# Peterande/SAST

Measured on AMD Instinct MI355X. Metric: frames/sec (B=4) SAST backbone fwd+bwd, 1Mpx 640x360, higher is better.
Workload: dtype f32; 1 GPU; 1Mpx 640x360 (padded 384x640) full SAST backbone + PAFPN, fwd+bwd + AdamW, B=4/GPU, binary events (rand>0.5), random-init, AMP=0.0002; global_batch=4, seq_len=1, parallelism=dp1, hipgraph=True, library=sast_amd/libsast_hip.so, product_library=True, segmented_backward_overlap=False, deferred_weight_gradients=False, backward_cuts=3, dw_discard_TIMING_PROBE_gradients_invalid=False, collective_ranks=1, collective_ranks_verified=1, gradient_bytes_per_rank=67663616, sync_batchnorm=False, event_dtype=int32, grads_finite=True

## Files before the change

### include/sast_hip.h

```cpp
#ifndef SAST_HIP_H
#define SAST_HIP_H
#include <stddef.h>
#include <stdint.h>

#ifdef __cplusplus
extern "C" {
#endif

typedef void* sast_stream_t;

enum { SAST_DT_F32 = 0, SAST_DT_I32 = 1, SAST_DT_U8 = 2, SAST_DT_I64 = 3, SAST_DT_I16 = 4, SAST_DT_I8 = 5 };

int sast_version(void);
int sast_mfma_split3(void);

int sast_nzratio(const void* x, int dtype, int B, int Cin, int H, int W, int32_t* cnt_ws, float* r, sast_stream_t stream);
int sast_nzratio_padded(const void* x, int dtype, int B, int Cin, int H, int W, int Hp, int Wp, int32_t* cnt_ws, float* r,
                        sast_stream_t stream);

int sast_input_prep(const void* x, int dtype, int B, int C, int H, int W, int Hp, int Wp, int32_t* ws, float* r, float* y,
                    sast_stream_t stream);
int sast_input_prep_flag(const void* x, int dtype, int B, int C, int H, int W, int Hp, int Wp, int32_t* ws, float* r, float* y,
                         uint32_t* nonexact, sast_stream_t stream);
int sast_input_prep_u8(const uint8_t* x, int B, int C, int H, int W, int Hp, int Wp, int32_t* ws, float* r, uint8_t* y, sast_stream_t stream);
// ... 33 lines not shown
typedef struct SastScoreArgs {
  int32_t B, L, C, r_stride;
  float amp;
  const float* xp;
  const float* r;
  const float* ws_w; const float* ws_b;
  const float* wc;
  float* scale;
  float* s;
  float* xw;
  float* tok;
  const float* dxw; float* dxp;
  float* d_ws_w; float* d_ws_b; float* d_wc;
  float* ws;
  float* dscale_ws;
} SastScoreArgs;
int sast_score_stp_fwd(const SastScoreArgs* a, sast_stream_t stream);
int sast_score_stp_bwd(const SastScoreArgs* a, sast_stream_t stream);

typedef struct SastSel {
  int32_t* win_keep;
  uint64_t* mask;
  int32_t* K;
  int32_t* row_off;
  int32_t* win_rank;
  int32_t* counts;
  int32_t* tok_slot;
  int32_t* row_tok;
  int32_t* pack_rows;
  int32_t* row_seg;
// ... 18 lines not shown
  float *mean1, *rstd1;
  float *mean2, *rstd2;
  float *S, *QKV, *O, *lse, *Y, *UG, *Hh;
  const float* dout; float* dxin;
  float *d_ln1_w, *d_ln1_b, *d_ln2_w, *d_ln2_b, *d_qkv_w, *d_qkv_b, *d_proj_w, *d_proj_b, *d_ls1;
  float *d_fc1_w, *d_fc1_b, *d_fc2_w, *d_fc2_b, *d_ls2;
  float* ws;
  float *cb_m, *cb_sum;
  float* raw_ws;
  const float *drop1, *drop2;
  float* drop_ws;
  const float* drop_mlp;
  float* fused_ws;
  const float* act_w;
  float* d_act_w;
} SastMswsaArgs;
size_t sast_mswsa_fused_ws_floats(int C, int inner, int T, int dim_head, int cb_tps);
size_t sast_mswsa_raw_ws_floats(int C, int inner);
size_t sast_mswsa_bwd_ws_floats(int rows, int C, int inner);
int sast_mswsa_fwd(const SastMswsaArgs* a, sast_stream_t stream);
int sast_mswsa_bwd(const SastMswsaArgs* a, sast_stream_t stream);

typedef struct SastLstmArgs {
  int32_t B, L, C;
  const float* x; const float* h0; const float* c0;
  const float* w; const float* b;
  float* h1; float* c1;
  float* gates;
  const float* dh1; const float* dc1;
  float* dx; float* dh0; float* dc0;
// ... 399 lines not shown
```

### sast_amd/csrc/k_block.hip

```cpp
#include <cstdlib>
#include "gemm_dispatch.cuh"
#include "kernels.h"

using namespace sast;

namespace {

constexpr int ATTN_MAX_T = 256;

struct EpBiasRelu {
  float* c; int ldc; const float* bias;
  struct Col { float b; };
  using Aux = EpNone;
  __device__ __forceinline__ Col col(int j) const { return Col{bias[j]}; }
  __device__ __forceinline__ Aux pre(int, int) const { return Aux{}; }
  __device__ __forceinline__ void post(int m, int j, const float (&v)[1], const Col& k, const Aux&) const {
    c[(size_t)m * ldc + j] = fmaxf(v[0] + k.b, 0.f);
  }
};
struct EpBiasReluCtl : EpBiasRelu {
  static constexpr bool SIDE = true;
  ControlsJob k; int side_blocks;
  __device__ __forceinline__ void side(int sb) const { if (threadIdx.x < 256) controls_fwd_elem(k, sb * 256 + threadIdx.x); }
};
// ... 297 lines not shown
  EpBiasReluCtl ep{};
  ep.c = a->s; ep.ldc = C; ep.bias = a->ws_b;
  ep.k = ControlsJob{a->wc, a->r, a->r_stride, a->scale, a->dscale_ws, nullptr, nullptr, a->B, C, 20};
  ep.side_blocks = (a->B * C + 255) / 256;
  int rc = gemm_auto(LdRows{a->xp, C, nullptr}, LdWeightNT{a->ws_w, C, 0}, ep, M, C, C, nullptr, st);
  if (rc) return rc;
  return stp_fwd_launch(a->xp, a->s, a->scale, a->amp, a->xw, a->tok, a->B, a->L, C, st);
}

int sast_score_stp_bwd(const SastScoreArgs* a, sast_stream_t stream) { SAST_ENTRY();
  hipStream_t st = (hipStream_t)stream;
  ProfScope ps_("score_bwd", a->C, a->B * a->L, st);
  const int M = a->B * a->L, C = a->C;
  float* dz = a->ws;
  float* dscale = a->dscale_ws ? a->dscale_ws : a->ws + (size_t)M * C;
  if (!a->dscale_ws) zero_fill(dscale, sizeof(float) * a->B * C, st);
  int rc = stp_bwd_launch(a->xp, a->s, a->scale, a->dxw, a->dxp, dz, dscale, a->B, a->L, C, st);
  if (rc) return rc;
  EpStoreAddCtl ep{};
  ep.c = a->dxp; ep.ldc = C; ep.add = a->dxp; ep.ldadd = C;
  ep.k = ControlsJob{a->wc, a->r, a->r_stride, nullptr, nullptr, dscale, a->d_wc, a->B, C, 20};
  ep.side_blocks = (C * 20 + 255) / 256;
  return gemm_pair(LdRowsT{dz, C}, LdRowsT{a->xp, C}, a->d_ws_w, C, C, C, M, nullptr, a->d_ws_b,
                   LdRows{dz, C, nullptr}, LdWeightNN{a->ws_w, C}, ep, M, C, C, nullptr, st);
}

size_t sast_mswsa_fused_ws_floats(int C, int inner, int T, int dim_head, int cb_tps) {
  const int on = SAST_KNOB("SAST_MSWSA_FUSED", 1);
  if (!on || !mswsa_fused_supported(C, inner, T, dim_head > 0 ? dim_head : 32, cb_tps)) return 0;
  return mswsa_fused_plane_floats(C, inner);
}
size_t sast_mswsa_raw_ws_floats(int C, int inner) { return (size_t)C * inner + (size_t)C * C + 2 * C; }

// ... 52 lines not shown
  if (!a->cb_m || !a->cb_sum || R % a->cb_tps) return SAST_EINVAL;
  rc = gemm_auto(LdRows{a->Hh, inner, nullptr}, LdWeightNT{a->fc2_w, inner, 0}, EpStore{a->cb_m, C, a->fc2_b}, R, C, inner, dR, st);
  if (rc) return rc;
  rc = cb_sample_sum_launch(a->cb_m, C, false, a->sel.row_tok, dR, R, a->cb_tps, R / a->cb_tps, C, a->cb_sum, st);
  if (rc) return rc;
  return cb_apply_fwd_launch(a->cb_m, a->Y, a->ls2, a->cb_sum, a->sel.row_tok, dR, R, a->cb_tps, C, a->out, st, a->drop2);
}

int sast_mswsa_bwd(const SastMswsaArgs* a, sast_stream_t stream) { SAST_ENTRY();
  hipStream_t st = (hipStream_t)stream;
  ProfScope ps_("mswsa_bwd", a->C, (a->mode ? -1 : 1) * a->B * a->H * a->W, st);
  const int C = a->C, L = a->H * a->W, R = a->B * L, inner = a->inner;
  const int T = a->ph * a->pw, NW = a->B * (L / T);
  const int dh = a->dim_head > 0 ? a->dim_head : 32;
  if (T > ATTN_MAX_T || a->mlp_act < 0 || a->mlp_act >= GLU_ACT_COUNT) return SAST_EINVAL;
  const int* dR = a->sel.counts;
  const int* row_tok = a->sel.row_tok;
  float* dUG = a->ws;
  float* dY = dUG + (size_t)R * 2 * inner;
  float* dO = dY + (size_t)R * C;
  float* dQKV = dO + (size_t)R * C;
  float* dS = dQKV + (size_t)R * 3 * C;
  float* raw2 = a->raw_ws ? a->raw_ws : dS + (size_t)R * C;
  float* raw1 = raw2 + (size_t)C * inner;
  float* s2 = raw1 + (size_t)C * C;
  float* s1 = s2 + C;
  if (!a->raw_ws) zero_fill(raw2, sizeof(float) * sast_mswsa_raw_ws_floats(C, inner), st);
  int rc;
  const float* dz = a->dout;
  const int* dz_tok = row_tok;
// ... 54 lines not shown
    rc = gemm_tn(LdRowsT{dYb, C}, LdRowsT{a->O, C}, raw1, C, C, C, R, dR, s1, st);
    if (rc) return rc;
    rc = gemm_auto(LdRows{dYb, C, nullptr}, LdWeightNN{a->proj_w, C}, EpStore{dO, C, nullptr}, R, C, C, dR, st);
  }
  if (rc) return rc;
  {
    const LsFinish f2{a->fc2_w, a->fc2_b, a->ls2, raw2, s2, a->d_fc2_w, a->d_fc2_b, a->d_ls2, inner};
    const LsFinish f1{a->proj_w, a->proj_b, a->ls1, raw1, s1, a->d_proj_w, a->d_proj_b, a->d_ls1, C};
    rc = attn_bwd_mfma_launch(a->QKV, dO, a->lse, dQKV, a->sel.row_off, a->sel.K, NW, T, C, dh, st, &f2, &f1, C,
                              a->ws + mswsa_bwd_ws_base(R, C, inner));
  }
  if (rc) return rc;
  rc = gemm_pair(LdRowsT{dQKV, 3 * C}, LdRowsT{a->S, C}, a->d_qkv_w, C, 3 * C, C, R, dR, a->d_qkv_b,
                 LdRows{dQKV, 3 * C, nullptr}, LdWeightNN{a->qkv_w, C}, EpStoreAdd{dS, C, dY, C}, R, C, 3 * C, dR, st);
  if (rc) return rc;
  return ln1_gather_bwd_launch(a->xin, a->dout, dS, a->sel.tok_slot, a->ln1_w, a->ln1_b, a->ln2_w, a->mean1, a->rstd1, a->mean2,
                               a->rstd2, a->dxin, a->d_ln1_w, a->d_ln1_b, a->d_ln2_w, a->d_ln2_b, R, C, st);
}

int sast_lstm_fwd(const SastLstmArgs* a, sast_stream_t stream) { SAST_ENTRY();
  hipStream_t st = (hipStream_t)stream;
  ProfScope ps_("lstm_fwd", a ? a->C : 0, a ? a->B * a->L : 0, st);
  if (!a || a->C % 4) return SAST_EINVAL;
  const int M = a->B * a->L, C = a->C;
  const int Kred = a->h0 ? 2 * C : C;
  const LdRows2 la{a->x, C, C, a->h0, C};
  const LdWeightNT lb{a->w, 2 * C, C};
  const EpLstm ep{a->b, a->c0, a->h1, a->c1, a->gates, C, a->drop};
  const int mode = SAST_KNOB("SAST_LSTM_TILE", 0);
  const bool k4 = mode && Kred >= 256 && (long)((M + 63) / 64) * ((C + 31) / 32) <= 2 * pair_thin_nb();
// ... 37 lines not shown
```

### sast_amd/csrc/k_rows.hip

```cpp
#include <cstdlib>
#include "common.cuh"
#include "kernels.h"

namespace sast {

__global__ __launch_bounds__(256) void zero_fill_kernel(float* __restrict__ p, size_t n) {
  const size_t i = (size_t)blockIdx.x * 256 + threadIdx.x;
  if (i < n) p[i] = 0.f;
}
int zero_fill(void* p, size_t bytes, hipStream_t st) {
  const size_t n = (bytes + 3) / 4;
  if (!n) return SAST_OK;
  SAST_LAUNCH(zero_fill_kernel, dim3((unsigned)((n + 255) / 256)), dim3(256), 0, st, (float*)p, n);
  SAST_CHECK_LAUNCH();
  return SAST_OK;
}

template <typename T>
__global__ __launch_bounds__(256) void nzr_count_kernel(const T* __restrict__ x, int* __restrict__ cnt, int C, int H, int W) {
  __shared__ float cell[8][33];
  const int plane = blockIdx.z;
  const int cy = threadIdx.x >> 5, cx = threadIdx.x & 31;
  const int y0 = blockIdx.y * 32 + cy * 4;
  int n1 = 0, n2 = 0, n3 = 0, n4 = 0;
// ... 450 lines not shown
    case 512: { constexpr int GL = 64, VPL = 2; CALL; } break;  \
    case 1024:{ constexpr int GL = 64, VPL = 4; CALL; } break;  \
    default: return SAST_EINVAL;                      \
  }

static int row_width_rc(int C) {
  SAST_DISPATCH_C(C, (void)(GL + VPL));
  return SAST_OK;
}
bool row_width_supported(int C) { return row_width_rc(C) == SAST_OK; }

static inline int bwd_grid(int rows, int rpb) {
  const int cap = SAST_KNOB("SAST_LN_BLOCKS", 256);
  int g = (rows + rpb - 1) / rpb;
  return g < 1 ? 1 : (g > cap ? cap : g);
}

int ln_fwd_launch(const float* x, float* y, const float* gamma, const float* beta, const float* add, int add_rows,
                  float* mean, float* rstd, int rows, int C, float eps, hipStream_t st) {
  if (rows <= 0) return SAST_OK;
  SAST_DISPATCH_C(C, SAST_LAUNCH((ln_fwd_kernel<GL, VPL>), dim3((rows + 256 / GL - 1) / (256 / GL)), dim3(256), 0, st,
                                        x, y, gamma, beta, add, add_rows, mean, rstd, rows, eps));
  SAST_CHECK_LAUNCH();
  return SAST_OK;
}

int ln_bwd_launch(const float* x, const float* dy, const float* gamma, const float* mean, const float* rstd, float* dx,
                  float* dgamma, float* dbeta, int rows, int C, hipStream_t st) {
  if (rows <= 0) return SAST_OK;
  SAST_DISPATCH_C(C, SAST_LAUNCH((ln_bwd_kernel<GL, VPL>), dim3(bwd_grid(rows, ROWB / GL)), dim3(ROWB),
// ... 20 lines not shown
  IO::load(xin + (size_t)row * IO::C, v, gl);
  IO::load(g1, gm, gl);
  IO::load(b1, bt, gl);
  float mean, rstd;
  ln_row<GL, VPL>(v, gm, bt, eps, mean, rstd);
  if (gl == 0) { mean1[row] = mean; rstd1[row] = rstd; }
  const int slot = tok_slot[row];
  if (slot < 0) { IO::store(out + (size_t)row * IO::C, v, gl); return; }
  IO::load(g2, gm, gl);
  IO::load(b2, bt, gl);
  ln_row<GL, VPL>(v, gm, bt, eps, mean, rstd);
  IO::store(sc + (size_t)slot * IO::C, v, gl);
  if (gl == 0) { mean2[slot] = mean; rstd2[slot] = rstd; }
}

template <int GL, int VPL>
__global__ __launch_bounds__(ROWB) void ln1_gather_bwd_kernel(const float* __restrict__ xin, const float* __restrict__ dout,
                                                             const float* __restrict__ dsc, const int* __restrict__ tok_slot,
                                                             const float* __restrict__ g1, const float* __restrict__ b1,
                                                             const float* __restrict__ g2,
                                                             const float* __restrict__ mean1, const float* __restrict__ rstd1,
                                                             const float* __restrict__ mean2, const float* __restrict__ rstd2,
                                                             float* __restrict__ dxin, float* __restrict__ dg1, float* __restrict__ db1,
                                                             float* __restrict__ dg2, float* __restrict__ db2, int rows) {
  SAST_KERNARG_WARM_SELF(ln1_gather_bwd_kernel<GL, VPL>);
  using IO = RowIO<GL, VPL>;
  extern __shared__ float red[];
  const int gl = threadIdx.x % GL;
  constexpr int RPB = ROWB / GL;
  float4 gm1[VPL], bt1[VPL], gm2[VPL], a1[VPL], c1[VPL], a2[VPL], c2[VPL];
  IO::load(g1, gm1, gl);
  IO::load(b1, bt1, gl);
  IO::load(g2, gm2, gl);
#pragma unroll
  for (int i = 0; i < VPL; ++i) { a1[i] = zero4(); c1[i] = zero4(); a2[i] = zero4(); c2[i] = zero4(); }
  for (int row = blockIdx.x * RPB + threadIdx.x / GL; row < rows; row += gridDim.x * RPB) {
    float4 xv[VPL], dv[VPL];
    IO::load(xin + (size_t)row * IO::C, xv, gl);
    const float m1 = mean1[row], r1 = rstd1[row];
    const int slot = tok_slot[row];
    if (slot >= 0) {
      float4 x1[VPL];
#pragma unroll
      for (int i = 0; i < VPL; ++i)
        x1[i] = make_float4((xv[i].x - m1) * r1 * gm1[i].x + bt1[i].x, (xv[i].y - m1) * r1 * gm1[i].y + bt1[i].y,
                            (xv[i].z - m1) * r1 * gm1[i].z + bt1[i].z, (xv[i].w - m1) * r1 * gm1[i].w + bt1[i].w);
      IO::load(dsc + (size_t)slot * IO::C, dv, gl);
      ln_row_bwd<GL, VPL>(x1, dv, gm2, mean2[slot], rstd2[slot], a2, c2);
    } else {
      IO::load(dout + (size_t)row * IO::C, dv, gl);
    }
    ln_row_bwd<GL, VPL>(xv, dv, gm1, m1, r1, a1, c1);
    IO::store(dxin + (size_t)row * IO::C, dv, gl);
  }
  flush_channel_partials<GL, VPL>(red, a1, dg1);
  flush_channel_partials<GL, VPL>(red, c1, db1);
  flush_channel_partials<GL, VPL>(red, a2, dg2);
  flush_channel_partials<GL, VPL>(red, c2, db2);
}

int ln1_gather_fwd_launch(const float* xin, float* out, float* sc, const int* tok_slot, const float* g1, const float* b1,
                          const float* g2, const float* b2, float* mean1, float* rstd1, float* mean2, float* rstd2,
                          int rows, int C, float eps, float* zero_ptr, size_t zero_floats, hipStream_t st) {
  SAST_DISPATCH_C(C, SAST_LAUNCH((ln1_gather_fwd_kernel<GL, VPL>), dim3((rows + 256 / GL - 1) / (256 / GL)), dim3(256), 0,
                                        st, xin, out, sc, tok_slot, g1, b1, g2, b2, mean1, rstd1, mean2, rstd2, rows, eps, zero_ptr,
                                        zero_ptr ? zero_floats / 4 : (size_t)0));
  SAST_CHECK_LAUNCH();
  return SAST_OK;
}

int ln1_gather_bwd_launch(const float* xin, const float* dout, const float* dsc, const int* tok_slot, const float* g1,
                          const float* b1, const float* g2, const float* mean1, const float* rstd1, const float* mean2,
                          const float* rstd2, float* dxin, float* dg1, float* db1, float* dg2, float* db2, int rows, int C,
                          hipStream_t st) {
  SAST_DISPATCH_C(C, SAST_LAUNCH((ln1_gather_bwd_kernel<GL, VPL>), dim3(bwd_grid(rows, ROWB / GL)), dim3(ROWB),
                                        sizeof(float) * (ROWB / GL) * C, st, xin, dout, dsc, tok_slot, g1, b1, g2, mean1, rstd1,
                                        mean2, rstd2, dxin, dg1, db1, dg2, db2, rows));
  SAST_CHECK_LAUNCH();
  return SAST_OK;
}

__global__ void controls_fwd_kernel(ControlsJob k) { controls_fwd_elem(k, blockIdx.x * blockDim.x + threadIdx.x); }
__global__ void controls_bwd_kernel(ControlsJob k) { controls_bwd_elem(k, blockIdx.x * blockDim.x + threadIdx.x); }

template <int GL, int VPL>
__global__ __launch_bounds__(256) void stp_fwd_kernel(const float* __restrict__ xp, const float* __restrict__ s,
                                                      const float* __restrict__ scale, float amp, float* __restrict__ xw,
                                                      float* __restrict__ tok, int rows, int L) {
  using IO = RowIO<GL, VPL>;
  const int gl = threadIdx.x % GL;
  const int row = (blockIdx.x * 256 + threadIdx.x) / GL;
  if (row >= rows) return;
// ... 514 lines not shown
```

### sast_amd/csrc/kernels.h

```cpp
#pragma once
#include <hip/hip_runtime.h>
#include "../../include/sast_hip.h"

namespace sast {

int zero_fill(void* p, size_t bytes, hipStream_t st);
int nzr_dispatch(const void* x, int dtype, int* cnt, float* r, int B, int C, int H, int W, int Hp, int Wp, hipStream_t st);
int nchw_to_nhwc_dispatch(const void* x, int dtype, float* y, int B, int C, int H, int W, int Hp, int Wp, hipStream_t st);
int input_prep_dispatch(const void* x, int dtype, float* y, int* ws, float* r, int B, int C, int H, int W, int Hp, int Wp, hipStream_t st,
                        unsigned* nonexact = nullptr);
int input_prep_u8(const unsigned char* x, unsigned char* y, int* ws, float* r, int B, int C, int H, int W, int Hp, int Wp, hipStream_t st);
int nhwc_to_nchw_launch(const float* x, float* y, int B, int C, int HW, hipStream_t st);
bool row_width_supported(int C);
int ln_fwd_launch(const float* x, float* y, const float* gamma, const float* beta, const float* add, int add_rows,
                  float* mean, float* rstd, int rows, int C, float eps, hipStream_t st);
int ln_bwd_launch(const float* x, const float* dy, const float* gamma, const float* mean, const float* rstd, float* dx,
                  float* dgamma, float* dbeta, int rows, int C, hipStream_t st);
int ln1_gather_fwd_launch(const float* xin, float* out, float* sc, const int* tok_slot, const float* g1, const float* b1,
                          const float* g2, const float* b2, float* mean1, float* rstd1, float* mean2, float* rstd2,
                          int rows, int C, float eps, float* zero_ptr, size_t zero_floats, hipStream_t st);
int ln1_gather_bwd_launch(const float* xin, const float* dout, const float* dsc, const int* tok_slot, const float* g1,
                          const float* b1, const float* g2, const float* mean1, const float* rstd1, const float* mean2,
                          const float* rstd2, float* dxin, float* dg1, float* db1, float* dg2, float* db2, int rows, int C,
                          hipStream_t st);
int controls_fwd_launch(const float* wc, const float* r, int r_stride, float* scale, int B, int C, int J, float* zero_bc,
                        hipStream_t st);
int controls_bwd_launch(const float* wc, const float* r, int r_stride, const float* dscale, float* dwc, int B, int C, int J,
                        hipStream_t st);
int stp_fwd_launch(const float* xp, const float* s, const float* scale, float amp, float* xw, float* tok, int B, int L, int C,
                   hipStream_t st);
int stp_bwd_launch(const float* xp, const float* s, const float* scale, const float* g, float* direct, float* dz,
                   float* dscale, int B, int L, int C, hipStream_t st);
int add_rows_launch(const float* x, const float* t, float* y, int rows, int C, int table_rows, hipStream_t st);
int row_scale_launch(const float* src, const int* idx, const float* rs, float* dst, const int* nrows_dev, int rows_max, int C, hipStream_t st);
int mask_token_fwd_launch(float* x, const unsigned char* mask, const float* token, const float* pe, int rows, int C, int L, hipStream_t st);
int mask_token_bwd_launch(const float* dy, const unsigned char* mask, float* dx, float* dtoken, int rows, int C, hipStream_t st);
int colsum_launch(const float* x, int ld, const int* idx, int rows, const int* drows, int C, float* out, hipStream_t st);
int mean_square_launch(const float* const* x, float* const* dx, const size_t* n, int count, int blocks, float* partials,
                       const float* g, int g_stride, hipStream_t st);
// ... 47 lines not shown
```

### sast_amd/functional.py

```python
from __future__ import annotations

import collections
import ctypes as C
import os
from typing import Dict, Optional, Tuple

import torch

from . import _lib as L

_DT = {torch.float32: L.DT_F32, torch.int32: L.DT_I32, torch.uint8: L.DT_U8, torch.int8: L.DT_I8}


_raw_stream = getattr(torch._C, "_cuda_getCurrentRawStream", None)


def _stream():
    if _raw_stream is not None:
        return C.c_void_p(_raw_stream(torch.cuda.current_device()))
    return C.c_void_p(torch.cuda.current_stream().cuda_stream)


def _need_gpu(*ts):
    for t in ts:
# ... 341 lines not shown
    def backward(ctx, dy):
        (m,) = ctx.saved_tensors
        dy = dy.contiguous()
        dx = torch.empty_like(dy)
        Cc = dy.shape[-1]
        pg = _ParamGrads(ctx.token)
        L.check(L.lib().sast_mask_token_bwd(dy.data_ptr(), m.data_ptr(), dx.data_ptr(), pg[0].data_ptr(), dy.numel() // Cc, Cc, _stream()),
                "mask_token_bwd")
        return dx, None, pg.out()[0], None


def mask_token(x_nhwc, token_mask, token, pos_emb_table=None):
    return _MaskToken.apply(x_nhwc, token_mask, token, pos_emb_table)


class _ScoreSTP(torch.autograd.Function):
    @staticmethod
    def forward(ctx, xp, r, ws_w, ws_b, wc, amp):
        _need_gpu(xp, r, ws_w)
        ctx.set_materialize_grads(False)
        xp = xp.contiguous()
        B = xp.shape[0]
        Cc = xp.shape[-1]
        Lt = xp.numel() // (B * Cc)
        assert r.shape[-1] == 20 and r.stride(-1) == 1
        dev = xp.device
        scale = torch.empty(B, Cc, device=dev)
        s = torch.empty(B * Lt, Cc, device=dev)
        xw = torch.empty_like(xp)
        tok = torch.empty(B, Lt, device=dev)
        dscale = torch.empty(B, Cc, device=dev)
        a = _fill(L.SastScoreArgs(), B=B, L=Lt, C=Cc, r_stride=r.stride(0), amp=amp, xp=xp, r=r, ws_w=ws_w, ws_b=ws_b, wc=wc,
                  scale=scale, s=s, xw=xw, tok=tok, dscale_ws=dscale)
        L.check(L.lib().sast_score_stp_fwd(C.byref(a), _stream()), "score_stp_fwd")
        ctx.save_for_backward(xp, r, scale, s, dscale)
        ctx.params = (ws_w, ws_b, wc)
        ctx.meta = (B, Lt, Cc, amp)
        ctx.mark_non_differentiable(tok)
        return xw, tok

    @staticmethod
    def backward(ctx, dxw, _dtok):
        xp, r, scale, s, dscale = ctx.saved_tensors
        ws_w, ws_b, wc = ctx.params
        B, Lt, Cc, amp = ctx.meta
        if dxw is None:
            return None, None, None, None, None, None
        _consume(ctx, "score_stp")
        dxw = dxw.contiguous()
        dxp = torch.empty_like(xp)
        ws = torch.empty(B * Lt * Cc + B * Cc, device=xp.device)
        pg = _ParamGrads(ws_w, ws_b, wc)
        a = _fill(L.SastScoreArgs(), B=B, L=Lt, C=Cc, r_stride=r.stride(0), amp=amp, xp=xp, r=r, ws_w=ws_w, ws_b=ws_b, wc=wc,
                  scale=scale, s=s, dxw=dxw, dxp=dxp, d_ws_w=pg[0], d_ws_b=pg[1], d_wc=pg[2], ws=ws, dscale_ws=dscale)
        L.check(L.lib().sast_score_stp_bwd(C.byref(a), _stream()), "score_stp_bwd")
        return (dxp, None) + pg.out() + (None,)


def score_stp(xp, r, ws_w, ws_b, wc, amp) -> Tuple[torch.Tensor, torch.Tensor]:
    return _ScoreSTP.apply(xp, r, ws_w, ws_b, wc, float(amp))


def mask_words(T: int) -> int:
    if T > 256:
        raise NotImplementedError("sast_amd: partitions of more than 256 tokens are not supported by the selection kernels")
    return 2 if T <= 128 else 4


class Selection:

    def __init__(self, B, H, W, ph, pw, mode, device):
        self.B, self.H, self.W, self.ph, self.pw, self.mode = B, H, W, ph, pw, mode
        self.T = ph * pw
        self.N = (H // ph) * (W // pw)
        self.L = H * W
# ... 162 lines not shown
        return f"DeviceCount({len(self.terms)} terms)"


_MSWSA_PARAMS = ("ln1_w", "ln1_b", "ln2_w", "ln2_b", "qkv_w", "qkv_b", "proj_w", "proj_b", "ls1",
                 "fc1_w", "fc1_b", "fc2_w", "fc2_b", "ls2", "act_w")


_FUSED_ENABLE = True
FUSED_MIN_ROWS_DEFAULT = int(os.environ.get("SAST_MSWSA_FUSED_MIN_ROWS", "49152"))
_FUSED_MIN_ROWS = FUSED_MIN_ROWS_DEFAULT
MSWSA_FORM_CALLS = {"fused": 0, "chain": 0}


class _MSWSA(torch.autograd.Function):
    @staticmethod
    def forward(ctx, xin, sel: Selection, eps, cb_tps, dim_head, fused, mlp_act, drop, grad_on, *params):
        _need_gpu(xin)
        xin = xin.contiguous()
        p = dict(zip(_MSWSA_PARAMS, params))
        Cc = xin.shape[-1]
        R = xin.numel() // Cc
        inner = p["fc2_w"].shape[1]
        if Cc % dim_head:
            raise RuntimeError(f"sast_amd: dim ({Cc}) must be a multiple of dim_head ({dim_head})")
        heads = Cc // dim_head
        dev = xin.device
        out = torch.empty_like(xin)
        a = L.SastMswsaArgs()
        _fill(a, B=sel.B, H=sel.H, W=sel.W, C=Cc, ph=sel.ph, pw=sel.pw, mode=sel.mode, inner=inner, eps=eps, dim_head=dim_head, mlp_act=mlp_act, xin=xin, out=out)
        sel.fill_struct(a.sel)
        _fill(a, **{k: _ptr(v) for k, v in p.items()})
# ... 34 lines not shown
            off += R * width
            return t

        S, QKV, O, Y, UG, Hh, lse = carve(Cc), carve(3 * Cc), carve(Cc), carve(Cc), carve(2 * inner), carve(inner), carve(heads)
        raw = torch.empty(L.lib().sast_mswsa_raw_ws_floats(Cc, inner), device=dev)
        _fill(a, raw_ws=raw, mean1=stats[0], rstd1=stats[1], mean2=stats[2], rstd2=stats[3], S=S, QKV=QKV, O=O, lse=lse, Y=Y, UG=UG, Hh=Hh)
        if cb_tps:
            if R % cb_tps:
                raise RuntimeError(f"sast_amd: Context Broadcasting needs rows ({R}) divisible by tokens per sample ({cb_tps})")
            cb_m, cb_sum = torch.empty(R, Cc, device=dev), torch.empty(R // cb_tps, Cc, device=dev)
            _fill(a, cb_tps=cb_tps, cb_m=cb_m, cb_sum=cb_sum)
        L.check(L.lib().sast_mswsa_fwd(C.byref(a), _stream()), "mswsa_fwd")
        ctx.save_for_backward(xin, stats, big, raw, fws)
        ctx.sel, ctx.params, ctx.eps, ctx.inner, ctx.cb_tps, ctx.dim_head, ctx.mlp_act = sel, params, eps, inner, cb_tps, dim_head, mlp_act
        ctx.drop, ctx.drop_mlp = drop, drop_mlp
        return out

    @staticmethod
    def backward(ctx, dout):
        xin, stats, big, raw, fws = ctx.saved_tensors
        _consume(ctx, "mswsa")
        sel, params, inner = ctx.sel, ctx.params, ctx.inner
        p = dict(zip(_MSWSA_PARAMS, params))
        Cc = xin.shape[-1]
        R = xin.numel() // Cc
        heads = Cc // ctx.dim_head
        dout = dout.contiguous()
        dxin = torch.empty_like(xin)
        flat = big.view(-1)
        off = 0

        def carve(width):
            nonlocal off
            t = flat[off:off + R * width]
            off += R * width
            return t

        S, QKV, O, Y, UG, Hh, lse = carve(Cc), carve(3 * Cc), carve(Cc), carve(Cc), carve(2 * inner), carve(inner), carve(heads)
        ws = torch.empty(L.lib().sast_mswsa_bwd_ws_floats(R, Cc, inner), device=xin.device)
        a = L.SastMswsaArgs()
        _fill(a, B=sel.B, H=sel.H, W=sel.W, C=Cc, ph=sel.ph, pw=sel.pw, mode=sel.mode, inner=inner, eps=ctx.eps, dim_head=ctx.dim_head, mlp_act=ctx.mlp_act, xin=xin,
              mean1=stats[0], rstd1=stats[1], mean2=stats[2], rstd2=stats[3], S=S, QKV=QKV, O=O, lse=lse, Y=Y, UG=UG, Hh=Hh,
              dout=dout, dxin=dxin, ws=ws, raw_ws=raw)
        if fws is not None:
            _fill(a, fused_ws=fws)
        if ctx.drop is not None:
            drop_ws = torch.empty(2 * R * Cc, device=xin.device)
            _fill(a, drop1=ctx.drop[0], drop2=ctx.drop[1], drop_ws=drop_ws)
        if ctx.drop_mlp is not None:
            _fill(a, drop_mlp=ctx.drop_mlp)
        if ctx.cb_tps:
            cb_m, cb_sum = torch.empty(R, Cc, device=xin.device), torch.empty(R // ctx.cb_tps, Cc, device=xin.device)
            _fill(a, cb_tps=ctx.cb_tps, cb_m=cb_m, cb_sum=cb_sum)
        sel.fill_struct(a.sel)
        _fill(a, **{k: _ptr(v) for k, v in p.items()})
        pg = _ParamGrads(*params)
        _fill(a, **{"d_" + k: _ptr(pg[i]) for i, k in enumerate(_MSWSA_PARAMS)})
        L.check(L.lib().sast_mswsa_bwd(C.byref(a), _stream()), "mswsa_bwd")
        return (dxin, None, None, None, None, None, None, None, None) + pg.out()


GLU_ACTIVATIONS = {"gelu": 0, "relu": 1, "silu": 2, "swish": 2, "sigmoid": 3, "tanh": 4, "mish": 5, "relu6": 6, "leaky_relu": 7, "elu": 8,
                   "celu": 8, "selu": 9, "hard_sigmoid": 10, "hardsigmoid": 10, "hard_swish": 11, "hardswish": 11, "hard_mish": 12, "prelu": 13}


def mswsa(xin, sel: Selection, eps: float, params: dict, cb_tokens_per_sample: int = 0, dim_head: int = 32, fused: bool = True,
          mlp_activation: str = "gelu", drop_path=None) -> torch.Tensor:
    if mlp_activation not in GLU_ACTIVATIONS:
        raise NotImplementedError(f"sast_amd: mlp_activation {mlp_activation!r}: the GLU epilogues implement {sorted(GLU_ACTIVATIONS)}")
    return _MSWSA.apply(xin, sel, float(eps), int(cb_tokens_per_sample), int(dim_head), bool(fused), GLU_ACTIVATIONS[mlp_activation],
                        drop_path, torch.is_grad_enabled(), *[params.get(k) if k == "act_w" else params[k] for k in _MSWSA_PARAMS])


class _LSTM(torch.autograd.Function):
    @staticmethod
    def forward(ctx, x, h0, c0, w, b, drop=None):
        _need_gpu(x, w)
        ctx.set_materialize_grads(False)
        x = x.contiguous()
        h0 = h0.contiguous() if h0 is not None else None
        c0 = c0.contiguous() if c0 is not None else None
        Cc = x.shape[-1]
        B = x.shape[0]
        Lt = x.numel() // (B * Cc)
        h1, c1 = torch.empty_like(x), torch.empty_like(x)
        gates = torch.empty(B * Lt, 4 * Cc, device=x.device)
# ... 960 lines not shown
```

### sast_amd/layers/sast.py

```python
from __future__ import annotations

import math
from typing import List, Optional, Tuple

import torch
from torch import nn

from .. import functional as SF
from .ops import LayerNorm, LayerScale, MLP, cfg_get


class PositiveLinear(nn.Module):

    def __init__(self, in_features, out_features, bias=True):
        super().__init__()
        self.in_features, self.out_features = in_features, out_features
        self.weight = nn.Parameter(torch.empty(out_features, in_features))
        if bias:
            self.bias = nn.Parameter(torch.empty(out_features))
        else:
            self.register_parameter('bias', None)
        self.reset_parameters()

    def reset_parameters(self):
# ... 96 lines not shown
                    ls2=getattr(self.ls2, "gamma", None), act_w=getattr(getattr(self.mlp.net[0], "act_layer", None), "weight", None))

    def _drop_path_factors(self, rows: int, device):
        if not self.training:
            return None
        if self.drop_path_override is not None:
            return self.drop_path_override
        dp, pm = isinstance(self.drop1, DropPath), self.mlp.net[1].p
        if not dp and pm == 0.0:
            return None
        d1 = self.drop1.row_factors(rows, device) if dp else None
        mask = torch.empty(rows, self.mlp.inner_dim, device=device).bernoulli_(1.0 - pm).div_(1.0 - pm) if pm > 0.0 else None
        d2 = self.drop2.row_factors(rows, device) if dp else None
        return d1, d2, mask

    def forward_image(self, x: torch.Tensor, sel: SF.Selection, enable_CB: bool = False, fused: bool = True) -> torch.Tensor:
        return SF.mswsa(x, sel, self.norm1.eps, self.kernel_params(), x.shape[1] * x.shape[2] if enable_CB else 0, self.dim_head, fused,
                        self.mlp_activation, self._drop_path_factors(x.numel() // x.shape[-1], x.device))

    def forward(self, x: torch.Tensor, index_window: torch.Tensor, index_token: torch.Tensor, padding_index: torch.Tensor,
                asy_index: torch.Tensor, M: int, B, enable_CB: bool) -> torch.Tensor:
        shape = x.shape
        N, C = x.shape[0], x.shape[-1]
        x3 = x.reshape(N, -1, C)
        T = x3.shape[1]
        K = torch.bincount(torch.div(asy_index, T, rounding_mode='floor'), minlength=len(index_window)) if len(index_window) \
            else torch.zeros(0, dtype=torch.long, device=x.device)
        sel = SF.selection_from_index_lists(index_window, asy_index, K, N, T, x.device)
        out = SF.mswsa(x3.reshape(1, N * T, 1, C), sel, self.norm1.eps, self.kernel_params(), N * T // int(B) if enable_CB else 0, self.dim_head,
                       mlp_activation=self.mlp_activation, drop_path=self._drop_path_factors(N * T, x.device))
        return out.view(*shape)


# ... 42 lines not shown
        self.sync_index_count = sync_index_count
        self.B, self.N, self.dim = None, None, dim

    def forward_posadded(self, xp: torch.Tensor, r: torch.Tensor, index_list):
        B, H, W, C = xp.shape
        ph, pw = self.partition_size
        self.B, self.N = B, H * W // (ph * pw)
        if self.first_block:
            xw, tok = SF.score_stp(xp, r, self.to_scores.weight, self.to_scores.bias, self.to_controls.weight, self.amp_value)
            sel1, sel2 = SF.select_pair(tok, B, H, W, ph, pw, self.bounce_value)
        else:
            xw = xp
            sel1, sel2 = index_list
            if not isinstance(sel1, SF.Selection):
                raise TypeError("sast_amd: index_list must be the [Selection, Selection] pair returned by the first block")
        x = self.win_attn.forward_image(xw, sel1, self.enable_CB, self.fused_forward)
        x = self.grid_attn.forward_image(x, sel2, self.enable_CB, self.fused_forward)
        count = SF.DeviceCount((sel1.counts[2], sel2.counts[2]))
        if self.sync_index_count:
            count = count.item()
        return x, count, [sel1, sel2]

    def forward(self, x: torch.Tensor, pos_emb, r: torch.Tensor, index_list) -> Tuple[torch.Tensor, object, List]:
        table = pos_emb.table_for(x) if hasattr(pos_emb, "table_for") else pos_emb(x)[0]
        xp = SF.add_pos_embedding(x, table.contiguous())
        return self.forward_posadded(xp, r, index_list)
```

Baseline: 890.1 frames/s.

## Fold score STP backward row pass into MSWSA ln1 gather backward kernel

When the first block's window attention is the only consumer of the score/STP output, its LN1 gather backward kernel now also computes the STP row-wise backward: the direct gradient into xp, dz for the score GEMM, and per-sample dscale partials. The kernel grid gains a per-sample dimension so dscale can be reduced per batch element. The separate stp_bwd launch, its zero fill, and one full read/write pass of a dxw tensor are then skipped in score_stp_bwd. The cost is a more complex kernel with Python handle plumbing and a check that xw has no other gradient consumer.

```diff
diff --git a/include/sast_hip.h b/include/sast_hip.h
--- a/include/sast_hip.h
+++ b/include/sast_hip.h
@@ -71,6 +71,7 @@
   float* d_ws_w; float* d_ws_b; float* d_wc;
   float* ws;
   float* dscale_ws;
+  int32_t rows_done;
 } SastScoreArgs;
 int sast_score_stp_fwd(const SastScoreArgs* a, sast_stream_t stream);
 int sast_score_stp_bwd(const SastScoreArgs* a, sast_stream_t stream);
@@ -119,6 +120,9 @@
   float* fused_ws;
   const float* act_w;
   float* d_act_w;
+  const float *stp_xp, *stp_s, *stp_scale;
+  float *stp_direct, *stp_dz, *stp_dscale;
+  int32_t stp_L;
 } SastMswsaArgs;
 size_t sast_mswsa_fused_ws_floats(int C, int inner, int T, int dim_head, int cb_tps);
 size_t sast_mswsa_raw_ws_floats(int C, int inner);
diff --git a/sast_amd/csrc/k_block.hip b/sast_amd/csrc/k_block.hip
--- a/sast_amd/csrc/k_block.hip
+++ b/sast_amd/csrc/k_block.hip
@@ -335,9 +335,13 @@
   const int M = a->B * a->L, C = a->C;
   float* dz = a->ws;
   float* dscale = a->dscale_ws ? a->dscale_ws : a->ws + (size_t)M * C;
-  if (!a->dscale_ws) zero_fill(dscale, sizeof(float) * a->B * C, st);
-  int rc = stp_bwd_launch(a->xp, a->s, a->scale, a->dxw, a->dxp, dz, dscale, a->B, a->L, C, st);
-  if (rc) return rc;
+  if (a->rows_done) {
+    if (!a->dscale_ws) return SAST_EINVAL;
+  } else {
+    if (!a->dscale_ws) zero_fill(dscale, sizeof(float) * a->B * C, st);
+    int rc = stp_bwd_launch(a->xp, a->s, a->scale, a->dxw, a->dxp, dz, dscale, a->B, a->L, C, st);
+    if (rc) return rc;
+  }
   EpStoreAddCtl ep{};
   ep.c = a->dxp; ep.ldc = C; ep.add = a->dxp; ep.ldadd = C;
   ep.k = ControlsJob{a->wc, a->r, a->r_stride, nullptr, nullptr, dscale, a->d_wc, a->B, C, 20};
@@ -420,6 +424,7 @@
   const int T = a->ph * a->pw, NW = a->B * (L / T);
   const int dh = a->dim_head > 0 ? a->dim_head : 32;
   if (T > ATTN_MAX_T || a->mlp_act < 0 || a->mlp_act >= GLU_ACT_COUNT) return SAST_EINVAL;
+  if (a->stp_xp && (!a->stp_s || !a->stp_scale || !a->stp_direct || !a->stp_dz || !a->stp_dscale || a->stp_L != L)) return SAST_EINVAL;
   const int* dR = a->sel.counts;
   const int* row_tok = a->sel.row_tok;
   float* dUG = a->ws;
@@ -504,6 +509,11 @@
   rc = gemm_pair(LdRowsT{dQKV, 3 * C}, LdRowsT{a->S, C}, a->d_qkv_w, C, 3 * C, C, R, dR, a->d_qkv_b,
                  LdRows{dQKV, 3 * C, nullptr}, LdWeightNN{a->qkv_w, C}, EpStoreAdd{dS, C, dY, C}, R, C, 3 * C, dR, st);
   if (rc) return rc;
+  if (a->stp_xp) {
+    const StpFold f{a->stp_xp, a->stp_s, a->stp_scale, a->stp_direct, a->stp_dz, a->stp_dscale};
+    return ln1_gather_bwd_launch(a->xin, a->dout, dS, a->sel.tok_slot, a->ln1_w, a->ln1_b, a->ln2_w, a->mean1, a->rstd1, a->mean2,
+                                 a->rstd2, nullptr, a->d_ln1_w, a->d_ln1_b, a->d_ln2_w, a->d_ln2_b, R, C, st, &f, a->B);
+  }
   return ln1_gather_bwd_launch(a->xin, a->dout, dS, a->sel.tok_slot, a->ln1_w, a->ln1_b, a->ln2_w, a->mean1, a->rstd1, a->mean2,
                                a->rstd2, a->dxin, a->d_ln1_w, a->d_ln1_b, a->d_ln2_w, a->d_ln2_b, R, C, st);
 }
diff --git a/sast_amd/csrc/k_rows.hip b/sast_amd/csrc/k_rows.hip
--- a/sast_amd/csrc/k_rows.hip
+++ b/sast_amd/csrc/k_rows.hip
@@ -488,6 +488,11 @@
   const int cap = SAST_KNOB("SAST_LN_BLOCKS", 256);
   int g = (rows + rpb - 1) / rpb;
   return g < 1 ? 1 : (g > cap ? cap : g);
+}
+static inline int bwd_grid_per_sample(int rows, int B, int rpb) {
+  const int per = bwd_grid(rows, rpb) / B, need = (rows / B + rpb - 1) / rpb;
+  const int g = per > need ? need : per;
+  return g < 1 ? 1 : g;
 }
 
 int ln_fwd_launch(const float* x, float* y, const float* gamma, const float* beta, const float* add, int add_rows,
@@ -538,7 +543,7 @@
   if (gl == 0) { mean2[slot] = mean; rstd2[slot] = rstd; }
 }
 
-template <int GL, int VPL>
+template <int GL, int VPL, bool STP>
 __global__ __launch_bounds__(ROWB) void ln1_gather_bwd_kernel(const float* __restrict__ xin, const float* __restrict__ dout,
                                                              const float* __restrict__ dsc, const int* __restrict__ tok_slot,
                                                              const float* __restrict__ g1, const float* __restrict__ b1,
@@ -546,19 +551,33 @@
                                                              const float* __restrict__ mean1, const float* __restrict__ rstd1,
                                                              const float* __restrict__ mean2, const float* __restrict__ rstd2,
                                                              float* __restrict__ dxin, float* __restrict__ dg1, float* __restrict__ db1,
-                                                             float* __restrict__ dg2, float* __restrict__ db2, int rows) {
-  SAST_KERNARG_WARM_SELF(ln1_gather_bwd_kernel<GL, VPL>);
+                                                             float* __restrict__ dg2, float* __restrict__ db2, int L, StpFold f) {
+  SAST_KERNARG_WARM_SELF(ln1_gather_bwd_kernel<GL, VPL, STP>);
   using IO = RowIO<GL, VPL>;
   extern __shared__ float red[];
   const int gl = threadIdx.x % GL;
   constexpr int RPB = ROWB / GL;
+  const int b = blockIdx.y;
   float4 gm1[VPL], bt1[VPL], gm2[VPL], a1[VPL], c1[VPL], a2[VPL], c2[VPL];
+  constexpr bool HOLD = VPL == 1;
+  float4 sc[STP && HOLD ? VPL : 1], ds[STP ? VPL : 1];
+  auto sig_scale = [&](float4 (&o)[VPL]) {
+    IO::load(f.scale + (size_t)b * IO::C, o, gl);
+#pragma unroll
+    for (int i = 0; i < VPL; ++i) o[i] = make_float4(sigmoid_hw(o[i].x), sigmoid_hw(o[i].y), sigmoid_hw(o[i].z), sigmoid_hw(o[i].w));
+  };
   IO::load(g1, gm1, gl);
   IO::load(b1, bt1, gl);
   IO::load(g2, gm2, gl);
 #pragma unroll
   for (int i = 0; i < VPL; ++i) { a1[i] = zero4(); c1[i] = zero4(); a2[i] = zero4(); c2[i] = zero4(); }
-  for (int row = blockIdx.x * RPB + threadIdx.x / GL; row < rows; row += gridDim.x * RPB) {
+  if constexpr (STP) {
+#pragma unroll
+    for (int i = 0; i < VPL; ++i) ds[i] = zero4();
+    if constexpr (HOLD) sig_scale(sc);
+  }
+  for (int l = blockIdx.x * RPB + threadIdx.x / GL; l < L; l += gridDim.x * RPB) {
+    const int row = b * L + l;
     float4 xv[VPL], dv[VPL];
     IO::load(xin + (size_t)row * IO::C, xv, gl);
     const float m1 = mean1[row], r1 = rstd1[row];
@@ -575,12 +594,45 @@
       IO::load(dout + (size_t)row * IO::C, dv, gl);
     }
     ln_row_bwd<GL, VPL>(xv, dv, gm1, m1, r1, a1, c1);
-    IO::store(dxin + (size_t)row * IO::C, dv, gl);
+    if constexpr (STP) {
+      float4 sv[VPL], zv[VPL];
+      IO::load(f.xp + (size_t)row * IO::C, xv, gl);
+      IO::load(f.s + (size_t)row * IO::C, sv, gl);
+      if constexpr (!HOLD) sig_scale(zv);
+#pragma unroll
+      for (int i = 0; i < VPL; ++i) {
+        const float* xs = &xv[i].x; const float* ss = &sv[i].x; float* gs = &dv[i].x; float* dd = &zv[i].x;
+        const float* cs = HOLD ? &sc[i].x : &zv[i].x; float* da = &ds[i].x;
+#pragma unroll
+        for (int e = 0; e < 4; ++e) {
+          const float sg = sigmoid_hw(ss[e]);
+          const float gx = gs[e] * xs[e];
+          const float ce = cs[e];
+          dd[e] = ss[e] > 0.f ? gx * ce * sg * (1.f - sg) : 0.f;
+          da[e] += gx * sg;
+          gs[e] = gs[e] * ce * sg;
+        }
+      }
+      IO::store(f.direct + (size_t)row * IO::C, dv, gl);
+      IO::store(f.dz + (size_t)row * IO::C, zv, gl);
+    } else {
+      IO::store(dxin + (size_t)row * IO::C, dv, gl);
+    }
   }
   flush_channel_partials<GL, VPL>(red, a1, dg1);
   flush_channel_partials<GL, VPL>(red, c1, db1);
   flush_channel_partials<GL, VPL>(red, a2, dg2);
   flush_channel_partials<GL, VPL>(red, c2, db2);
+  if constexpr (STP) {
+    float4 cf[VPL];
+    sig_scale(cf);
+#pragma unroll
+    for (int i = 0; i < VPL; ++i) {
+      ds[i].x *= cf[i].x * (1.f - cf[i].x); ds[i].y *= cf[i].y * (1.f - cf[i].y);
+      ds[i].z *= cf[i].z * (1.f - cf[i].z); ds[i].w *= cf[i].w * (1.f - cf[i].w);
+    }
+    flush_channel_partials<GL, VPL>(red, ds, f.dscale + (size_t)b * IO::C);
+  }
 }
 
 int ln1_gather_fwd_launch(const float* xin, float* out, float* sc, const int* tok_slot, const float* g1, const float* b1,
@@ -596,10 +648,19 @@
 int ln1_gather_bwd_launch(const float* xin, const float* dout, const float* dsc, const int* tok_slot, const float* g1,
                           const float* b1, const float* g2, const float* mean1, const float* rstd1, const float* mean2,
                           const float* rstd2, float* dxin, float* dg1, float* db1, float* dg2, float* db2, int rows, int C,
-                          hipStream_t st) {
-  SAST_DISPATCH_C(C, SAST_LAUNCH((ln1_gather_bwd_kernel<GL, VPL>), dim3(bwd_grid(rows, ROWB / GL)), dim3(ROWB),
+                          hipStream_t st, const StpFold* stp, int B) {
+  if (stp) {
+    if (B < 1 || rows % B) return SAST_EINVAL;
+    const int L = rows / B;
+    SAST_DISPATCH_C(C, SAST_LAUNCH((ln1_gather_bwd_kernel<GL, VPL, true>), dim3(bwd_grid_per_sample(rows, B, ROWB / GL), B), dim3(ROWB),
+                                          sizeof(float) * (ROWB / GL) * C, st, xin, dout, dsc, tok_slot, g1, b1, g2, mean1, rstd1,
+                                          mean2, rstd2, dxin, dg1, db1, dg2, db2, L, *stp));
+    SAST_CHECK_LAUNCH();
+    return SAST_OK;
+  }
+  SAST_DISPATCH_C(C, SAST_LAUNCH((ln1_gather_bwd_kernel<GL, VPL, false>), dim3(bwd_grid(rows, ROWB / GL)), dim3(ROWB),
                                         sizeof(float) * (ROWB / GL) * C, st, xin, dout, dsc, tok_slot, g1, b1, g2, mean1, rstd1,
-                                        mean2, rstd2, dxin, dg1, db1, dg2, db2, rows));
+                                        mean2, rstd2, dxin, dg1, db1, dg2, db2, rows, StpFold{}));
   SAST_CHECK_LAUNCH();
   return SAST_OK;
 }
diff --git a/sast_amd/csrc/kernels.h b/sast_amd/csrc/kernels.h
--- a/sast_amd/csrc/kernels.h
+++ b/sast_amd/csrc/kernels.h
@@ -19,10 +19,14 @@
 int ln1_gather_fwd_launch(const float* xin, float* out, float* sc, const int* tok_slot, const float* g1, const float* b1,
                           const float* g2, const float* b2, float* mean1, float* rstd1, float* mean2, float* rstd2,
                           int rows, int C, float eps, float* zero_ptr, size_t zero_floats, hipStream_t st);
+struct StpFold {
+  const float* xp; const float* s; const float* scale;
+  float* direct; float* dz; float* dscale;
+};
 int ln1_gather_bwd_launch(const float* xin, const float* dout, const float* dsc, const int* tok_slot, const float* g1,
                           const float* b1, const float* g2, const float* mean1, const float* rstd1, const float* mean2,
                           const float* rstd2, float* dxin, float* dg1, float* db1, float* dg2, float* db2, int rows, int C,
-                          hipStream_t st);
+                          hipStream_t st, const StpFold* stp = nullptr, int B = 1);
 int controls_fwd_launch(const float* wc, const float* r, int r_stride, float* scale, int B, int C, int J, float* zero_bc,
                         hipStream_t st);
 int controls_bwd_launch(const float* wc, const float* r, int r_stride, const float* dscale, float* dwc, int B, int C, int J,
diff --git a/sast_amd/functional.py b/sast_amd/functional.py
--- a/sast_amd/functional.py
+++ b/sast_amd/functional.py
@@ -379,9 +379,22 @@
     return _MaskToken.apply(x_nhwc, token_mask, token, pos_emb_table)
 
 
+class StpHandle:
+    __slots__ = ("xp", "s", "scale", "dscale", "B", "L", "dxp", "ws", "done")
+
+    def __init__(self):
+        self.xp = self.s = self.scale = self.dscale = self.dxp = self.ws = None
+        self.B = self.L = -1
+        self.done = False
+
+
+def stp_fold_bwd_enabled() -> bool:
+    return bool(L.lib().sast_config_get(b"SAST_STP_FOLD_BWD", 1))
+
+
 class _ScoreSTP(torch.autograd.Function):
     @staticmethod
-    def forward(ctx, xp, r, ws_w, ws_b, wc, amp):
+    def forward(ctx, xp, r, ws_w, ws_b, wc, amp, handle=None):
         _need_gpu(xp, r, ws_w)
         ctx.set_materialize_grads(False)
         xp = xp.contiguous()
@@ -402,6 +415,9 @@
         ctx.params = (ws_w, ws_b, wc)
         ctx.meta = (B, Lt, Cc, amp)
         ctx.mark_non_differentiable(tok)
+        ctx.stp = handle
+        if handle is not None:
+            handle.xp, handle.s, handle.scale, handle.dscale, handle.B, handle.L = xp, s, scale, dscale, B, Lt
         return xw, tok
 
     @staticmethod
@@ -409,21 +425,35 @@
         xp, r, scale, s, dscale = ctx.saved_tensors
         ws_w, ws_b, wc = ctx.params
         B, Lt, Cc, amp = ctx.meta
-        if dxw is None:
-            return None, None, None, None, None, None
+        h = ctx.stp
+        rows_done = h is not None and h.done
+        if dxw is None and not rows_done:
+            return None, None, None, None, None, None, None
         _consume(ctx, "score_stp")
-        dxw = dxw.contiguous()
-        dxp = torch.empty_like(xp)
-        ws = torch.empty(B * Lt * Cc + B * Cc, device=xp.device)
+        if rows_done:
+            dxp, ws = h.dxp, h.ws
+            h.dxp = h.ws = None
+            if dxw is not None and dxw.data_ptr() != dxp.data_ptr():
+                raise RuntimeError("sast_amd: score_stp: the layer that was declared the only consumer of xw folded the STP backward into its "
+                                   "own, but xw received a gradient from somewhere else as well")
+        else:
+            dxw = dxw.contiguous()
+            dxp = torch.empty_like(xp)
+            ws = torch.empty(B * Lt * Cc + B * Cc, device=xp.device)
         pg = _ParamGrads(ws_w, ws_b, wc)
         a = _fill(L.SastScoreArgs(), B=B, L=Lt, C=Cc, r_stride=r.stride(0), amp=amp, xp=xp, r=r, ws_w=ws_w, ws_b=ws_b, wc=wc,
-                  scale=scale, s=s, dxw=dxw, dxp=dxp, d_ws_w=pg[0], d_ws_b=pg[1], d_wc=pg[2], ws=ws, dscale_ws=dscale)
+                  scale=scale, s=s, dxw=_ptr(dxw), dxp=dxp, d_ws_w=pg[0], d_ws_b=pg[1], d_wc=pg[2], ws=ws, dscale_ws=dscale,
+                  rows_done=int(rows_done))
         L.check(L.lib().sast_score_stp_bwd(C.byref(a), _stream()), "score_stp_bwd")
-        return (dxp, None) + pg.out() + (None,)
+        return (dxp, None) + pg.out() + (None, None)
 
 
 def score_stp(xp, r, ws_w, ws_b, wc, amp) -> Tuple[torch.Tensor, torch.Tensor]:
-    return _ScoreSTP.apply(xp, r, ws_w, ws_b, wc, float(amp))
+    handle = StpHandle() if torch.is_grad_enabled() else None
+    xw, tok = _ScoreSTP.apply(xp, r, ws_w, ws_b, wc, float(amp), handle)
+    if handle is not None:
+        xw._sast_stp = handle
+    return xw, tok
 
 
 def mask_words(T: int) -> int:
@@ -616,7 +646,7 @@
 
 class _MSWSA(torch.autograd.Function):
     @staticmethod
-    def forward(ctx, xin, sel: Selection, eps, cb_tps, dim_head, fused, mlp_act, drop, grad_on, *params):
+    def forward(ctx, xin, sel: Selection, eps, cb_tps, dim_head, fused, mlp_act, drop, grad_on, stp, *params):
         _need_gpu(xin)
         xin = xin.contiguous()
         p = dict(zip(_MSWSA_PARAMS, params))
@@ -681,6 +711,7 @@
         ctx.save_for_backward(xin, stats, big, raw, fws)
         ctx.sel, ctx.params, ctx.eps, ctx.inner, ctx.cb_tps, ctx.dim_head, ctx.mlp_act = sel, params, eps, inner, cb_tps, dim_head, mlp_act
         ctx.drop, ctx.drop_mlp = drop, drop_mlp
+        ctx.stp = stp if (stp is not None and ctx.needs_input_grad[0]) else None
         return out
 
     @staticmethod
@@ -693,7 +724,13 @@
         R = xin.numel() // Cc
         heads = Cc // ctx.dim_head
         dout = dout.contiguous()
-        dxin = torch.empty_like(xin)
+        stp = ctx.stp if (ctx.stp is not None and not ctx.stp.done) else None
+        if stp is None:
+            dxin = torch.empty_like(xin)
+        else:
+            stp.dxp = torch.empty_like(stp.xp)
+            dxin = stp.dxp.view_as(xin)
+            stp.ws = torch.empty(R * Cc + stp.B * Cc, device=xin.device)
         flat = big.view(-1)
         off = 0
 
@@ -709,6 +746,8 @@
         _fill(a, B=sel.B, H=sel.H, W=sel.W, C=Cc, ph=sel.ph, pw=sel.pw, mode=sel.mode, inner=inner, eps=ctx.eps, dim_head=ctx.dim_head, mlp_act=ctx.mlp_act, xin=xin,
               mean1=stats[0], rstd1=stats[1], mean2=stats[2], rstd2=stats[3], S=S, QKV=QKV, O=O, lse=lse, Y=Y, UG=UG, Hh=Hh,
               dout=dout, dxin=dxin, ws=ws, raw_ws=raw)
+        if stp is not None:
+            _fill(a, stp_xp=stp.xp, stp_s=stp.s, stp_scale=stp.scale, stp_direct=stp.dxp, stp_dz=stp.ws, stp_dscale=stp.dscale, stp_L=stp.L)
         if fws is not None:
             _fill(a, fused_ws=fws)
         if ctx.drop is not None:
@@ -724,7 +763,9 @@
         pg = _ParamGrads(*params)
         _fill(a, **{"d_" + k: _ptr(pg[i]) for i, k in enumerate(_MSWSA_PARAMS)})
         L.check(L.lib().sast_mswsa_bwd(C.byref(a), _stream()), "mswsa_bwd")
-        return (dxin, None, None, None, None, None, None, None, None) + pg.out()
+        if stp is not None:
+            stp.done = True
+        return (dxin, None, None, None, None, None, None, None, None, None) + pg.out()
 
 
 GLU_ACTIVATIONS = {"gelu": 0, "relu": 1, "silu": 2, "swish": 2, "sigmoid": 3, "tanh": 4, "mish": 5, "relu6": 6, "leaky_relu": 7, "elu": 8,
@@ -732,11 +773,15 @@
 
 
 def mswsa(xin, sel: Selection, eps: float, params: dict, cb_tokens_per_sample: int = 0, dim_head: int = 32, fused: bool = True,
-          mlp_activation: str = "gelu", drop_path=None) -> torch.Tensor:
+          mlp_activation: str = "gelu", drop_path=None, stp_sole: bool = False) -> torch.Tensor:
     if mlp_activation not in GLU_ACTIVATIONS:
         raise NotImplementedError(f"sast_amd: mlp_activation {mlp_activation!r}: the GLU epilogues implement {sorted(GLU_ACTIVATIONS)}")
+    stp = getattr(xin, "_sast_stp", None) if stp_sole else None
+    if stp is not None and (AUTOGRAD_GRADS or not torch.is_grad_enabled() or not xin.is_contiguous() or stp.xp.numel() != xin.numel()
+                            or stp.B != sel.B or stp.L != sel.H * sel.W or not stp_fold_bwd_enabled()):
+        stp = None
     return _MSWSA.apply(xin, sel, float(eps), int(cb_tokens_per_sample), int(dim_head), bool(fused), GLU_ACTIVATIONS[mlp_activation],
-                        drop_path, torch.is_grad_enabled(), *[params.get(k) if k == "act_w" else params[k] for k in _MSWSA_PARAMS])
+                        drop_path, torch.is_grad_enabled(), stp, *[params.get(k) if k == "act_w" else params[k] for k in _MSWSA_PARAMS])
 
 
 class _LSTM(torch.autograd.Function):
diff --git a/sast_amd/layers/sast.py b/sast_amd/layers/sast.py
--- a/sast_amd/layers/sast.py
+++ b/sast_amd/layers/sast.py
@@ -134,9 +134,9 @@
         d2 = self.drop2.row_factors(rows, device) if dp else None
         return d1, d2, mask
 
-    def forward_image(self, x: torch.Tensor, sel: SF.Selection, enable_CB: bool = False, fused: bool = True) -> torch.Tensor:
+    def forward_image(self, x: torch.Tensor, sel: SF.Selection, enable_CB: bool = False, fused: bool = True, stp_sole: bool = False) -> torch.Tensor:
         return SF.mswsa(x, sel, self.norm1.eps, self.kernel_params(), x.shape[1] * x.shape[2] if enable_CB else 0, self.dim_head, fused,
-                        self.mlp_activation, self._drop_path_factors(x.numel() // x.shape[-1], x.device))
+                        self.mlp_activation, self._drop_path_factors(x.numel() // x.shape[-1], x.device), stp_sole=stp_sole)
 
     def forward(self, x: torch.Tensor, index_window: torch.Tensor, index_token: torch.Tensor, padding_index: torch.Tensor,
                 asy_index: torch.Tensor, M: int, B, enable_CB: bool) -> torch.Tensor:
@@ -209,7 +209,7 @@
             sel1, sel2 = index_list
             if not isinstance(sel1, SF.Selection):
                 raise TypeError("sast_amd: index_list must be the [Selection, Selection] pair returned by the first block")
-        x = self.win_attn.forward_image(xw, sel1, self.enable_CB, self.fused_forward)
+        x = self.win_attn.forward_image(xw, sel1, self.enable_CB, self.fused_forward, stp_sole=self.first_block)
         x = self.grid_attn.forward_image(x, sel2, self.enable_CB, self.fused_forward)
         count = SF.DeviceCount((sel1.counts[2], sel2.counts[2]))
         if self.sync_index_count:
```

Result: no change. 896.6 frames/s, median of 6 (+0.7%).
